# merlresearch/tssep

Measured on AMD Instinct MI355X. Metric: frames/sec fwd+bwd, 4-spk TS-SEP, 16kHz 4s chunks, higher is better.
Workload: dtype bf16x3+f32

## Files before the change

include/tssep_hip.h:

```cpp
#ifndef TSSEP_HIP_H
#define TSSEP_HIP_H

#include <stdint.h>

#ifdef __cplusplus
extern "C" {
#endif

#define TSSEP_OK 0
#define TSSEP_E_SHAPE (-1)
#define TSSEP_E_ALIGN (-2)
#define TSSEP_E_UNSUPPORTED (-3)
#define TSSEP_E_LAUNCH (-4)
#define TSSEP_E_NULL (-5)

int tssep_abi_version(void);
const char* tssep_arch(void);

int tssep_probe_mfma(float* out_4x4, float* out_32x32, void* stream);
int tssep_probe_xcc(int* out, int nblocks, void* stream);
int tssep_probe_clock(int64_t* out, int nblocks, int iters, int heavy, void* stream);
int tssep_probe_rewrite(float* buf, int nblocks, int bytes_per_wg, int reps, int flavour, int read_flavour,
                        const float* stream_src, int64_t stream_bytes, int pressure, float* sink, void* stream);

// ... 6 lines not shown
                   float* X, int64_t T, void* stream);

int64_t tssep_istft_chunks(int64_t N);
int tssep_istft_fwd(const float* X, int64_t rows, int64_t T, int size, int shift,
                    int fading, const float* wsyn, const float* tw,
                    float* y, int64_t N, const float* tgt, float* abs_partial, void* stream);
int tssep_istft_bwd(const float* dy, int64_t rows, int64_t N, int size, int shift,
                    int fading, const float* wsyn, const float* tw,
                    float* dX, int64_t T, void* stream);

int tssep_mask_istft_fwd(const float* logit, const float* obs, int64_t B, int64_t K, int64_t T,
                         int size, int shift, int fading, const float* wsyn, const float* tw,
                         float* y, int64_t N, const float* tgt, float* abs_partial, void* stream);
int tssep_mask_istft_bwd(const float* dy, const float* logit, const float* obs, int64_t B,
                         int64_t K, int64_t N, int size, int shift, int fading,
                         const float* wsyn, const float* tw, float* dlogit, int64_t T, void* stream);
int tssep_mask_istft_bwd_loss(const float* est, const float* tgt, const float* sums, const float* gout,
                              const float* logit, const float* obs, int64_t B, int64_t K, int64_t N,
                              int size, int shift, int fading, const float* wsyn, const float* tw,
                              const int32_t* iperm, int bt_major, float* dlogit, int64_t T, void* stream);
int tssep_mask_istft_gated_fwd(const float* logit, const float* obs, int64_t B, int64_t K, int64_t T, int size,
                               int shift, int fading, const float* wsyn, const float* tw, float* y, int64_t N,
                               const float* tgt, float* abs_partial, void* stream);
int tssep_mask_istft_gated_bwd(const float* est, const float* tgt, const float* sums, const float* gout,
                               const float* vad, const float* gout_vad, const float* logit, const float* obs,
                               int64_t B, int64_t K, int64_t N, int size, int shift, int fading,
                               const float* wsyn, const float* tw, const int32_t* iperm, int bt_major,
                               float* dlogit, int64_t T, void* stream);

int64_t tssep_feat_workspace_bytes(int64_t B, int64_t T, int n_mels, int F, int stat_axis);
int tssep_feat_fwd(const float* X, int64_t B, int64_t T, int F,
                   const float* fb, const float* dct, int n_mels, int n_mfcc,
                   float top_db, int stat_axis, float* out, int64_t ld_out, void* ws, void* stream);

typedef struct tssep_gemm_args {
  const float* A; const float* B; float* C;
  int64_t M, N, K;
  int64_t lda, ldb, ldc;
  int32_t a_kmajor, b_kmajor;
  int64_t b_kshift, kperiod;
  const float* bias;
  int32_t act;
  int32_t accumulate;
  int32_t c_remap;
  int64_t c_T, c_K, c_sb, c_sk, c_st, c_cm, c_co;
  const int32_t* c_perm; int64_t c_perm_ld;
  int32_t splitk; int64_t c_split_stride;
  int32_t precision;
  int32_t b_ones_col;
  const float* aux; int64_t ldaux;
} tssep_gemm_args;
int tssep_gemm_f32(const tssep_gemm_args* args, void* stream);

#define TSSEP_GEMM_AUTO 0
#define TSSEP_GEMM_F32 1
#define TSSEP_GEMM_PIPE 2
#define TSSEP_GEMM_TALL2 3
#define TSSEP_GEMM_TALL4 4
#define TSSEP_GEMM_TALL4_XCOL 5
#define TSSEP_GEMM_BIG 6
#define TSSEP_GEMM_STREAM 7
#define TSSEP_GEMM_NT_W160 8
#define TSSEP_GEMM_TN 9
#define TSSEP_GEMM_TN_TALL 10
#define TSSEP_GEMM_TN_BIG 11
#define TSSEP_GEMM_TN_W160 12
// ... 174 lines not shown
```

tssep_amd/csrc/feat.hip:

```cpp
#include <math.h>
#include "common.h"

namespace {

__device__ __forceinline__ unsigned ord(float f) {
  const unsigned u = __float_as_uint(f);
  return (u & 0x80000000u) ? ~u : (u | 0x80000000u);
}
__device__ __forceinline__ float unord(unsigned u) {
  return __uint_as_float((u & 0x80000000u) ? (u & 0x7fffffffu) : ~u);
}

constexpr int MAXF = 1032;
constexpr int GSLOTS = 64;

struct FeatWs {
  unsigned* gmax;
  unsigned* umax;
  int* range;
  float* fbT;
  float* db;
};
constexpr int STAT_TF = 0, STAT_T = 1, STAT_F = 2;
__host__ __device__ inline int64_t feat_nmax(int64_t B, int F, int stat) { return stat == STAT_T ? B * F : B; }
__host__ __device__ inline FeatWs feat_ws(void* ws, int64_t B , int n_mels) {
  FeatWs w;
  char* p = (char*)ws;
  w.gmax = (unsigned*)p;
  w.umax = (unsigned*)(p + GSLOTS * 4);
  const int64_t off1 = GSLOTS * 4 + ((B * 4 + 15) / 16) * 16;
  w.range = (int*)(p + off1);
  const int64_t off2 = off1 + (((int64_t)2 * n_mels * 4 + 15) / 16) * 16;
  w.fbT = (float*)(p + off2);
  w.db = (float*)(p + off2 + (int64_t)n_mels * MAXF * 4);
  return w;
}

__global__ __launch_bounds__(64) void feat_init_kernel(void* ws, int64_t B, const float* __restrict__ fb,
                                                       int F, int n_mels) {
  FeatWs w = feat_ws(ws, B, n_mels);
  const int lane = threadIdx.x, m = blockIdx.x;
  if (m == 0) w.gmax[lane] = 0u;
  for (int64_t b = (int64_t)m * 64 + lane; b < B; b += (int64_t)gridDim.x * 64) w.umax[b] = 0u;
  if (m >= n_mels) return;
  float lo = (float)F, hi = 0.f;
  for (int f = lane; f < F; f += 64) {
    const float v = fb[(int64_t)f * n_mels + m];
    w.fbT[(int64_t)m * MAXF + f] = v;
    if (v != 0.f) { lo = fminf(lo, (float)f); hi = fmaxf(hi, (float)(f + 1)); }
  }
  lo = -wave_max(-lo);
  hi = wave_max(hi);
  if (lane == 0) {
    w.range[2 * m] = hi == 0.f ? 0 : (int)lo;
    w.range[2 * m + 1] = (int)hi;
  }
}

constexpr int FPW = 4;
constexpr int CWMAX = 2 * MAXF;
constexpr int LMELS = 128;

__global__ __launch_bounds__(256) void feat_pass1_kernel(const float2* __restrict__ X, int64_t B,
                                                         int64_t T, int F,
                                                         const float* __restrict__ fb, int n_mels,
                                                         int n_mfcc, void* ws, int stat, int log_mels) {
  __shared__ float pw[4][MAXF];
  __shared__ float cw[CWMAX];
  __shared__ int clo[LMELS], chi[LMELS], coff[LMELS + 1];
  __shared__ int s_packed;
  FeatWs w = feat_ws(ws, feat_nmax(B, F, stat), n_mels);
  const int tid = threadIdx.x, lane = tid & 63, wave = tid >> 6;
  if (n_mfcc > 0) {
    if (tid < n_mels && tid < LMELS) {
      clo[tid] = w.range[2 * tid];
      chi[tid] = w.range[2 * tid + 1];
    }
    __syncthreads();
    if (tid == 0) {
      int tot = 0;
      const int nm = n_mels < LMELS ? n_mels : LMELS;
      for (int m = 0; m < nm; ++m) {
        coff[m] = tot;
        const int wd = chi[m] - clo[m];
        tot += wd > 0 ? wd : 0;
      }
      coff[nm] = tot;
      s_packed = (n_mels <= LMELS && tot <= CWMAX) ? 1 : 0;
    }
    __syncthreads();
    if (s_packed)
      for (int m = wave; m < n_mels; m += 4)
        for (int f = clo[m] + lane; f < chi[m]; f += 64) cw[coff[m] + f - clo[m]] = w.fbT[(int64_t)m * MAXF + f];
    __syncthreads();
  }
  const bool packed = n_mfcc > 0 && s_packed;
  float dbmax = -INFINITY;
  for (int it = 0; it < FPW; ++it) {
    const int64_t frame = ((int64_t)blockIdx.x * FPW + it) * 4 + wave;
    if (frame >= B * T) break;
    const float2* x = X + frame * F;
    float amax = 0.f;
    float2 xv[17];
#pragma unroll
    for (int r = 0; r < 17; ++r) {
      const int f = lane + 64 * r;
      xv[r] = f < F ? x[f] : make_float2(0.f, 0.f);
    }
#pragma unroll
    for (int r = 0; r < 17; ++r) {
      const int f = lane + 64 * r;
      if (f < F) {
        const float p = xv[r].x * xv[r].x + xv[r].y * xv[r].y;
        pw[wave][f] = p;
        amax = fmaxf(amax, sqrtf(p));
        if (stat == STAT_T) {
          unsigned* slot = w.umax + (frame / T) * F + f;
          const unsigned o_ = ord(sqrtf(p));
          if (o_ > __hip_atomic_load(slot, __ATOMIC_RELAXED, __HIP_MEMORY_SCOPE_AGENT)) atomicMax(slot, o_);
        }
      }
    }
    __builtin_amdgcn_fence(__ATOMIC_RELEASE, "wavefront");
    __builtin_amdgcn_wave_barrier();
    __builtin_amdgcn_fence(__ATOMIC_ACQUIRE, "wavefront");
    amax = wave_max(amax);
    if (lane == 0 && stat == STAT_TF) atomicMax(w.umax + frame / T, ord(amax));
    if (n_mfcc > 0) {
      for (int m0 = 0; m0 < n_mels; m0 += 64) {
        float mine = 0.f;
        const int mm = n_mels - m0 < 64 ? n_mels - m0 : 64;
        if (lane < mm) {
          const int m = m0 + lane;
          const int lo = packed ? clo[m] : w.range[2 * m], hi = packed ? chi[m] : w.range[2 * m + 1];
          const float* frow = packed ? cw + coff[m] - lo : w.fbT + (int64_t)m * MAXF;
          const float* prow = pw[wave];
          float s0 = 0.f, s1 = 0.f, s2 = 0.f, s3 = 0.f;
          int f = lo;
          for (; f + 3 < hi; f += 4) {
            s0 = fmaf(prow[f], frow[f], s0);
            s1 = fmaf(prow[f + 1], frow[f + 1], s1);
            s2 = fmaf(prow[f + 2], frow[f + 2], s2);
            s3 = fmaf(prow[f + 3], frow[f + 3], s3);
          }
          if (f < hi) s0 = fmaf(prow[f], frow[f], s0);
          if (f + 1 < hi) s1 = fmaf(prow[f + 1], frow[f + 1], s1);
          if (f + 2 < hi) s2 = fmaf(prow[f + 2], frow[f + 2], s2);
          mine = (s0 + s1) + (s2 + s3);
        }
        if (lane < mm) {
          const float db = log_mels ? logf(mine + 1e-6f) : 10.0f * log10f(fmaxf(mine, 1e-10f));
          w.db[frame * n_mels + m0 + lane] = db;
          dbmax = fmaxf(dbmax, db);
        }
      }
    }
    __builtin_amdgcn_fence(__ATOMIC_RELEASE, "wavefront");
    __builtin_amdgcn_wave_barrier();
    __builtin_amdgcn_fence(__ATOMIC_ACQUIRE, "wavefront");
  }
  if (n_mfcc > 0) {
    dbmax = wave_max(dbmax);
    if (lane == 0 && dbmax > -INFINITY) atomicMax(w.gmax + (blockIdx.x & (GSLOTS - 1)), ord(dbmax));
  }
}

__global__ __launch_bounds__(256) void feat_pass2_kernel(const float2* __restrict__ X, int64_t B,
                                                         int64_t T, int F,
                                                         const float* __restrict__ dct, int n_mels,
                                                         int n_mfcc, float top_db,
                                                         float* __restrict__ out, int64_t ld_out,
                                                         const void* ws, int stat) {
  __shared__ float dbl[4][64];
  FeatWs w = feat_ws(const_cast<void*>(ws), feat_nmax(B, F, stat), n_mels);
  const int lane = threadIdx.x & 63, wave = threadIdx.x >> 6;
  const int64_t frame = (int64_t)blockIdx.x * 4 + wave;
  const bool valid = frame < B * T;
  float* o = out + (valid ? frame : 0) * ld_out;
  if (n_mfcc > 0) {
    const float floor_db = top_db < 0.f ? -INFINITY : wave_max(unord(w.gmax[lane])) - top_db;
    for (int m0 = 0; m0 < n_mels; m0 += 64) {
      if (valid && m0 + lane < n_mels)
        dbl[wave][lane] = fmaxf(w.db[frame * n_mels + m0 + lane], floor_db);
      __syncthreads();
      if (valid) {
        const int mm = n_mels - m0 < 64 ? n_mels - m0 : 64;
        for (int c = lane; c < n_mfcc; c += 64) {
          float s = m0 ? o[c] : 0.f;
          for (int m = 0; m < mm; ++m) s = fmaf(dbl[wave][m], dct[(int64_t)(m0 + m) * n_mfcc + c], s);
          o[c] = s;
        }
      }
      __syncthreads();
    }
  }
  if (!valid) return;
  const float2* x = X + frame * F;
  float2 xv[17];
#pragma unroll
  for (int r = 0; r < 17; ++r) {
    const int f = lane + 64 * r;
    xv[r] = f < F ? x[f] : make_float2(0.f, 0.f);
  }
  if (stat == STAT_TF) {
    const float scale = (float)(M_E - 1.0) / unord(w.umax[frame / T]);
#pragma unroll
    for (int r = 0; r < 17; ++r) {
      const int f = lane + 64 * r;
      if (f < F) o[n_mfcc + f] = log1pf(sqrtf(xv[r].x * xv[r].x + xv[r].y * xv[r].y) * scale);
    }
    return;
  }
  float fmx = 0.f;
  if (stat == STAT_F) {
#pragma unroll
    for (int r = 0; r < 17; ++r)
      if (lane + 64 * r < F) fmx = fmaxf(fmx, sqrtf(xv[r].x * xv[r].x + xv[r].y * xv[r].y));
    fmx = wave_max(fmx);
  }
#pragma unroll
  for (int r = 0; r < 17; ++r) {
    const int f = lane + 64 * r;
    if (f < F) {
      const float norm = stat == STAT_F ? fmx : unord(w.umax[(frame / T) * F + f]);
      o[n_mfcc + f] = log1pf(sqrtf(xv[r].x * xv[r].x + xv[r].y * xv[r].y) * ((float)(M_E - 1.0) / norm));
    }
  }
}

}

extern "C" int64_t tssep_feat_workspace_bytes(int64_t B, int64_t T, int n_mels, int F, int stat_axis) {
  if (stat_axis < 0 || stat_axis > 2 || F <= 0) return 0;
  FeatWs w = feat_ws(nullptr, feat_nmax(B, F, stat_axis), n_mels);
  return (int64_t)((char*)w.db - (char*)nullptr) + B * T * (int64_t)n_mels * 4 + 16;
}

extern "C" int tssep_feat_fwd(const float* X, int64_t B, int64_t T, int F, const float* fb,
                              const float* dct, int n_mels, int n_mfcc, float top_db, int stat_axis,
                              float* out, int64_t ld_out, void* ws, void* stream) {
  if (!X || !out || !ws) return TSSEP_E_NULL;
  if (n_mfcc > 0 && (!fb || !dct)) return TSSEP_E_NULL;
  if (B <= 0 || T <= 0 || F <= 0 || F > MAXF || ld_out < n_mfcc + F) return TSSEP_E_SHAPE;
  if (n_mfcc > 0 && (n_mels <= 0 || n_mels > 1024)) return TSSEP_E_SHAPE;
  if (n_mfcc == 0) n_mels = 0;
  if (stat_axis < 0 || stat_axis > 2) return TSSEP_E_SHAPE;
  if ((((uintptr_t)X) & 7u) || (((uintptr_t)ws) & 15u)) return TSSEP_E_ALIGN;
  hipStream_t s = (hipStream_t)stream;
  const int nm = n_mels > 0 ? n_mels : 1;
  const int64_t nmax = feat_nmax(B, F, stat_axis);
  const int64_t nb0 = (nmax + 64 * 16 - 1) / (64 * 16);
  hipLaunchKernelGGL(feat_init_kernel, dim3((unsigned)(nb0 > nm ? (nb0 > 4096 ? 4096 : nb0) : nm)), dim3(64), 0, s, ws, nmax, fb, F, n_mels);
  const unsigned blocks = (unsigned)((B * T + 3) / 4);
  const unsigned blocks1 = (unsigned)((B * T + 4 * FPW - 1) / (4 * FPW));
  hipLaunchKernelGGL(feat_pass1_kernel, dim3(blocks1), dim3(256), 0, s, (const float2*)X, B, T, F,
                     fb, n_mels, n_mfcc, ws, stat_axis, top_db < 0.f ? 1 : 0);
  hipLaunchKernelGGL(feat_pass2_kernel, dim3(blocks), dim3(256), 0, s, (const float2*)X, B, T, F,
                     dct, n_mels, n_mfcc, top_db, out, ld_out, ws, stat_axis);
  return tssep_launch_status();
}
```

tssep_amd/csrc/stft.hip:

```cpp
#include <math.h>
#include "common.h"

namespace {

typedef __amdgpu_buffer_rsrc_t srd_t;
typedef unsigned u32x2_t __attribute__((ext_vector_type(2)));
__device__ __forceinline__ srd_t make_srd(const void* p, int64_t bytes) {
  return __builtin_amdgcn_make_buffer_rsrc(const_cast<void*>(p), 0, (int)(bytes > 0x7fffffff ? 0x7fffffff : bytes), 0x00020000);
}
__device__ __forceinline__ float2 bload2(srd_t r, unsigned voff) {
  const u32x2_t v = __builtin_amdgcn_raw_buffer_load_b64(r, (int)voff, 0, 0);
  return make_float2(__uint_as_float(v[0]), __uint_as_float(v[1]));
}

__device__ __forceinline__ float bload1(srd_t r, unsigned voff) {
  return __uint_as_float(__builtin_amdgcn_raw_buffer_load_b32(r, (int)voff, 0, 0));
}
__device__ __forceinline__ void bstore1(srd_t r, unsigned voff, float v) {
  __builtin_amdgcn_raw_buffer_store_b32(__float_as_uint(v), r, (int)voff, 0, 0);
}

constexpr int NH = 512;
constexpr int LINE = NH + NH / 8;
#define PADI(i) ((i) + ((i) >> 3))
#define WAVE_SYNC()                                          \
  do {                                                       \
    __builtin_amdgcn_fence(__ATOMIC_RELEASE, "wavefront");   \
    __builtin_amdgcn_wave_barrier();                         \
    __builtin_amdgcn_fence(__ATOMIC_ACQUIRE, "wavefront");   \
  } while (0)

__device__ __forceinline__ float2 cmul(float2 a, float2 b) {
  return make_float2(a.x * b.x - a.y * b.y, a.x * b.y + a.y * b.x);
}
// ... 36 lines not shown

__device__ __forceinline__ void fft512_wave(float2 (&v)[8], float2* buf, const float2* twl, int lane) {
  fft8(v);
#pragma unroll
  for (int r = 0; r < 8; ++r) buf[PADI(8 * lane + r)] = v[r];
  WAVE_SYNC();
#pragma unroll
  for (int r = 0; r < 8; ++r) v[r] = buf[PADI(lane + 64 * r)];
  WAVE_SYNC();
  {
    const int k = lane & 7;
#pragma unroll
    for (int r = 1; r < 8; ++r) v[r] = cmul(v[r], twl[k * r * 8]);
    fft8(v);
    const int d = (lane >> 3) * 64 + k;
#pragma unroll
    for (int r = 0; r < 8; ++r) buf[PADI(d + 8 * r)] = v[r];
  }
  WAVE_SYNC();
#pragma unroll
  for (int r = 0; r < 8; ++r) v[r] = buf[PADI(lane + 64 * r)];
  WAVE_SYNC();
#pragma unroll
  for (int r = 1; r < 8; ++r) v[r] = cmul(v[r], twl[lane * r]);
  fft8(v);
#pragma unroll
  for (int r = 0; r < 8; ++r) buf[PADI(lane + 64 * r)] = v[r];
  WAVE_SYNC();
}

#ifndef TSSEP_RFFT_OCC
#define TSSEP_RFFT_OCC 3
#endif
template <bool MASKED, bool GATED = false>
__global__ __launch_bounds__(256, TSSEP_RFFT_OCC) void rfft_frames_kernel(
    const float* __restrict__ x, int64_t rows, int64_t N, int64_t T, int shift, int pad_left,
    const float* __restrict__ window, const float2* __restrict__ tw, float2* __restrict__ X,
    float s_in, float s_edge, int iters, const float* __restrict__ logit,
    const float2* __restrict__ obs, float* __restrict__ dlogit, int64_t Kspk,
    const float* __restrict__ tgt, const float* __restrict__ sums, const float* __restrict__ gout,
    const int32_t* __restrict__ iperm, int bt_major, const float* __restrict__ vad = nullptr,
    const float* __restrict__ gbce = nullptr, float inv_kt = 0.f) {
  static_assert(MASKED || !GATED, "the gate belongs to the mask head");
  constexpr int LDL = NH + 1 + (GATED ? 1 : 0);
  constexpr int C0 = GATED ? 1 : 0;
  __shared__ float2 twl[NH];
  __shared__ float2 wl[NH];
  __shared__ float2 line[4][LINE];
  const int tid = threadIdx.x, lane = tid & 63;
  const int wave = __builtin_amdgcn_readfirstlane(tid >> 6);
  for (int i = tid; i < NH; i += 256) { twl[i] = tw[i]; wl[i] = reinterpret_cast<const float2*>(window)[i]; }
  __syncthreads();
  const float2 tw2_lane = tw[NH + lane];
  const int64_t total = rows * T;
  for (int it = 0; it < iters; ++it) {
    const int64_t fidx = ((int64_t)blockIdx.x * iters + it) * 4 + wave;
    const bool valid = fidx < total;
    const int64_t row = valid ? fidx / T : 0;
    const int64_t t = valid ? fidx - row * T : 0;
    const int64_t base = t * shift - pad_left;
    const float* xr = x + row * N;
    const bool lossgrad = MASKED && tgt != nullptr;
    const float* tr_ = lossgrad ? tgt + row * N : xr;
    float coef = 0.f;
    if (lossgrad) {
      const int64_t b = row / Kspk;
      coef = sums ? gout[b] / ((float)N * 2.30258509299404568402f * sums[b]) : gout[b] / (float)N;
    }
    auto lg = [&](float e, float t_) { const float d = e - t_; return d > 0.f ? coef : (d < 0.f ? -coef : 0.f); };
    const bool fast = ((N & 1) == 0) && ((base & 1) == 0) && ((((uintptr_t)x) & 7u) == 0) &&
                      (!lossgrad || (((uintptr_t)tgt) & 7u) == 0);
    float2 v[8];
    if (!valid) {
#pragma unroll
      for (int r = 0; r < 8; ++r) v[r] = make_float2(0.f, 0.f);
    } else if (fast) {
      const unsigned vo = (unsigned)((base + 2 * lane) * 4);
      const srd_t sx = make_srd(xr, N * 4);
      float2 xv[8];
#pragma unroll
      for (int r = 0; r < 8; ++r) xv[r] = bload2(sx, vo + 512u * r);
      if (lossgrad) {
        const srd_t st_ = make_srd(tr_, N * 4);
        float2 tv[8];
#pragma unroll
// ... 41 lines not shown
      for (int r = 0; r < 8; ++r) {
        ob8[r] = bload2(so, (unsigned)(lane * 8 + 512 * r));
        lg8[r] = bload1(sl, (unsigned)(C0 * 4 + lane * 4 + 256 * r));
      }
      if (GATED) lgate = bload1(sl, 0u);
    }
    fft512_wave(v, buf, twl, lane);
    if (valid) {
      float2* Xo = MASKED ? nullptr : X + fidx * (NH + 1);
      float* Dr = MASKED ? dlogit + fidx * LDL : nullptr;
      if (MASKED && bt_major) {
        const int64_t b = row / Kspk, j = row - b * Kspk;
        const int64_t kpos = iperm ? (int64_t)iperm[b * Kspk + j] : j;
        Dr = dlogit + ((b * T + t) * Kspk + kpos) * LDL;
      }
      const float gm = GATED ? sigmoidf_mask(lgate) : 1.f;
      float gpart = 0.f;
      auto emit = [&](int k, float2 o, float lgk, float2 ob) {
        if (GATED) {
          const float s = sigmoidf_mask(lgk);
          const float dm = ob.x * o.x + ob.y * o.y;
          Dr[C0 + k] = dm * gm * s * (1.0f - s);
          gpart += dm * s;
        } else if (MASKED) {
          const float m = sigmoidf_mask(lgk);
          Dr[k] = (ob.x * o.x + ob.y * o.y) * m * (1.0f - m);
        } else {
          Xo[k] = o;
        }
      };
      float2 wr[8];
      lane_twiddles(tw2_lane, wr);
      const float hs_in = 0.5f * s_in;
#pragma unroll
      for (int r = 0; r < 8; ++r) {
        const int k = lane + 64 * r;
        const float2 zk = buf[PADI(k)];
        const int km = (NH - k) & (NH - 1);
        float2 zm = buf[PADI(km)];
        zm.y = -zm.y;
        const float2 u = cmul(wr[r], csub(zk, zm));
        float2 o = make_float2(zk.x + zm.x + u.y, zk.y + zm.y - u.x);
        if (k == 0) {
          o.x *= 0.5f * s_edge; o.y = 0.f;
        } else {
          o.x *= hs_in; o.y *= hs_in;
        }
        emit(k, o, MASKED ? lg8[r] : 0.f, MASKED ? ob8[r] : make_float2(0.f, 0.f));
      }
      if (lane == 0) {
        const float2 z0 = buf[0];
        emit(NH, make_float2((z0.x - z0.y) * s_edge, 0.f), MASKED ? Lr[C0 + NH] : 0.f, MASKED ? Or[NH] : make_float2(0.f, 0.f));
      }
      if (GATED) {
        const float tot = wave_sum(gpart);
        if (lane == 0) {
          float dv = tot * gm * (1.0f - gm);
          if (vad) dv += gbv * (sigmoidf_acc(lgate) - vadv) * inv_kt;
          Dr[0] = dv;
        }
      }
    }
    WAVE_SYNC();
  }
}

constexpr int RING = 7;
constexpr int HCB_MAX = 64;

#ifndef TSSEP_ISTFT_OCC
#define TSSEP_ISTFT_OCC 3
#endif
template <bool MASKED, bool GATED = false>
__global__ __launch_bounds__(256, TSSEP_ISTFT_OCC) void istft_kernel(
    const float2* __restrict__ X, int64_t T, int shift_, int64_t N,
    const float* __restrict__ wsyn, const float2* __restrict__ tw, float* __restrict__ y,
    const float* __restrict__ tgt, float* __restrict__ abs_partial, int nchunks, int hcb,
    const float* __restrict__ logit, const float2* __restrict__ obs, int64_t Kspk) {
  __shared__ float2 twl[NH];
  __shared__ float2 line[4][LINE];
  __shared__ __attribute__((aligned(16))) float fr[RING][1024];
  __shared__ float red[4];
  static_assert(MASKED || !GATED, "the gate belongs to the mask head");
  constexpr int LDL = NH + 1 + (GATED ? 1 : 0);
  constexpr int C0 = GATED ? 1 : 0;
  const int tid = threadIdx.x, lane = tid & 63;
  const int wave = __builtin_amdgcn_readfirstlane(tid >> 6);
  const int64_t row = blockIdx.y;
  const int c = blockIdx.x;
  for (int i = tid; i < NH; i += 256) twl[i] = tw[i];
  __syncthreads();
  const float2 tw2_lane = tw[NH + lane];
  const int64_t t_lo = (int64_t)c * hcb;
  const int64_t n0 = t_lo * 256;
  const int64_t total_hops = (N + 255) / 256;
  const int hops = (int)(total_hops - t_lo < hcb ? total_hops - t_lo : hcb);
// ... 153 lines not shown
  }
  return TSSEP_OK;
}

static int check_plan(int size, int shift) {
  if (size != 1024 || shift != 256) return TSSEP_E_UNSUPPORTED;
  return TSSEP_OK;
}
static bool generic_plan(int size, int shift) { return check_plan(size, shift) != TSSEP_OK && tssep_generic_plan_supported(size, shift); }
extern "C" int tssep_stft_plan(int size, int shift) {
  return check_plan(size, shift) == TSSEP_OK ? 1 : (tssep_generic_plan_supported(size, shift) ? 2 : 0);
}

extern "C" int tssep_stft_fwd(const float* x, int64_t rows, int64_t N, int size, int shift,
                              int fading, const float* window, const float* tw, float* X,
                              int64_t T, void* stream) {
  if (!x || !window || !tw || !X) return TSSEP_E_NULL;
  if (rows <= 0 || N <= 0 || T <= 0) return TSSEP_E_SHAPE;
  if ((((uintptr_t)X) & 7u) || (((uintptr_t)tw) & 7u) || (((uintptr_t)window) & 7u)) return TSSEP_E_ALIGN;
  if (generic_plan(size, shift))
    return tssep_generic_rfft(x, rows, N, size, shift, fading ? size - shift : 0, window, tw, X, T, 1.0f, 1.0f, stream);
  if (int e = check_plan(size, shift)) return e;
  const int iters = 4;
  const int64_t total = rows * T;
  const int64_t blocks = (total + 4 * iters - 1) / (4 * iters);
  hipLaunchKernelGGL(rfft_frames_kernel<false>, dim3((unsigned)blocks), dim3(256), 0, (hipStream_t)stream,
                     x, rows, N, T, shift, fading ? size - shift : 0, window, (const float2*)tw,
                     (float2*)X, 1.0f, 1.0f, iters, (const float*)nullptr, (const float2*)nullptr,
                     (float*)nullptr, (int64_t)1, (const float*)nullptr, (const float*)nullptr,
                     (const float*)nullptr, (const int32_t*)nullptr, 0);
  return tssep_launch_status();
}

extern "C" int tssep_istft_bwd(const float* dy, int64_t rows, int64_t N, int size, int shift,
                               int fading, const float* wsyn, const float* tw, float* dX,
                               int64_t T, void* stream) {
  if (!dy || !wsyn || !tw || !dX) return TSSEP_E_NULL;
  if (rows <= 0 || N <= 0 || T <= 0) return TSSEP_E_SHAPE;
  if ((((uintptr_t)dX) & 7u) || (((uintptr_t)tw) & 7u) || (((uintptr_t)wsyn) & 7u)) return TSSEP_E_ALIGN;
  if (generic_plan(size, shift))
    return tssep_generic_rfft(dy, rows, N, size, shift, fading ? size - shift : 0, wsyn, tw, dX, T, 2.0f / (float)size,
                              1.0f / (float)size, stream);
  if (int e = check_plan(size, shift)) return e;
  const int iters = 4;
  const int64_t total = rows * T;
  const int64_t blocks = (total + 4 * iters - 1) / (4 * iters);
  hipLaunchKernelGGL(rfft_frames_kernel<false>, dim3((unsigned)blocks), dim3(256), 0, (hipStream_t)stream,
                     dy, rows, N, T, shift, fading ? size - shift : 0, wsyn, (const float2*)tw,
                     (float2*)dX, 2.0f / (float)size, 1.0f / (float)size, iters, (const float*)nullptr,
                     (const float2*)nullptr, (float*)nullptr, (int64_t)1, (const float*)nullptr, (const float*)nullptr,
                     (const float*)nullptr, (const int32_t*)nullptr, 0);
  return tssep_launch_status();
}

extern "C" int tssep_mask_istft_bwd(const float* dy, const float* logit, const float* obs, int64_t B,
                                    int64_t K, int64_t N, int size, int shift, int fading,
                                    const float* wsyn, const float* tw, float* dlogit, int64_t T,
                                    void* stream) {
  if (!dy || !logit || !obs || !wsyn || !tw || !dlogit) return TSSEP_E_NULL;
  if (B <= 0 || K <= 0 || N <= 0 || T <= 0) return TSSEP_E_SHAPE;
  if (int e = check_plan(size, shift)) return e;
  if ((((uintptr_t)obs) & 7u) || (((uintptr_t)tw) & 7u) || (((uintptr_t)wsyn) & 7u)) return TSSEP_E_ALIGN;
  const int iters = 4;
  const int64_t rows = B * K, total = rows * T;
  const int64_t blocks = (total + 4 * iters - 1) / (4 * iters);
  hipLaunchKernelGGL(rfft_frames_kernel<true>, dim3((unsigned)blocks), dim3(256), 0, (hipStream_t)stream,
// ... 117 lines not shown
```

tssep_amd/hip_ops.py:

```python
import ctypes
import itertools
import math

import numpy as np
import torch

from . import _lib
from ._lib import GemmArgs, LstmSizes, check


KERNEL_TIMING = False
KERNEL_TIMERS = {}
KERNEL_FLOPS = {}
KERNEL_BYTES = {}


class _timed:
    def __init__(self, name, flops=0, nbytes=0):
        self.name, self.flops, self.nbytes = name, flops, nbytes

    def __enter__(self):
        if KERNEL_TIMING:
            self.s = torch.cuda.Event(enable_timing=True)
            self.e = torch.cuda.Event(enable_timing=True)
# ... 222 lines not shown
    if vad is not None:
        v, gv = _f32(vad[0]).contiguous(), _f32(vad[1]).contiguous()
        assert tuple(v.shape) == (B, K, T) and gv.numel() == B, (tuple(v.shape), (B, K, T), gv.numel())
    with _timed("maskhead_gated_bwd", 0, B * T * (8 * K * F1 + 8 * (F1 - 1)) + 4 * B * K * x.shape[-1]):
        check(L.tssep_mask_istft_gated_bwd(_p(x), _p(tgt), _p(sums), _p(gout), _p(v), _p(gv), _p(logit), _p(obs_r),
                                           B, K, x.shape[-1], size, shift, int(fading), _p(wsyn),
                                           _p(fft_tables(size, logit.device)), _p(iperm), int(bt_major), _p(dlogit),
                                           T, _stream()), "mask_istft_gated_bwd")
    return dlogit


STAT_AXES = {"tf": 0, "t": 1, "f": 2}


def feat_fwd(X, fb, dct, n_mfcc, top_db=80.0, statistics_axis="tf"):
    L = _lib.lib()
    Xr = torch.view_as_real(X.contiguous())
    B, T, F = X.shape
    n_mels = fb.shape[1] if n_mfcc else 0
    if n_mfcc:
        fb, dct = _f32(fb).contiguous(), _f32(dct).contiguous()
    D = n_mfcc + F
    ld = round_up(D, 4)
    out = torch.empty(B, T, ld, device=X.device, dtype=torch.float32)
    if ld != D:
        out[..., D:].zero_()
    stat = STAT_AXES[statistics_axis]
    ws = torch.empty(int(L.tssep_feat_workspace_bytes(B, T, max(n_mels, 1), F, stat)) // 4 + 4,
                     device=X.device, dtype=torch.float32)
    check(L.tssep_feat_fwd(_p(Xr), B, T, F, _p(fb) if n_mfcc else None,
                           _p(dct) if n_mfcc else None, n_mels, n_mfcc, float(top_db), stat, _p(out),
                           ld, _p(ws), _stream()), "feat_fwd")
    return out[..., :D], ld


GEMM_PRECISION = "bf16x3"
_PREC = {"f32": 0, "bf16x3": 1, "bf16": 3}


def _gemm_args(A, lda, B, ldb, C, ldc, M, N, K, a_kmajor=False, b_kmajor=False, bias=None, act=0,
               accumulate=False, b_kshift=0, kperiod=0, remap=None, splitk=1, split_stride=0,
               b_ones_col=False, aux=None):
    def ptr(x):
        if isinstance(x, tuple):
            return x[0].data_ptr() + 4 * x[1]
        return x.data_ptr()
    g = GemmArgs()
    g.A, g.B, g.C = ptr(A), ptr(B), ptr(C)
    g.M, g.N, g.K = M, N, K
    g.lda, g.ldb, g.ldc = lda, ldb, ldc
    g.a_kmajor, g.b_kmajor = int(a_kmajor), int(b_kmajor)
    g.b_kshift, g.kperiod = b_kshift, kperiod
    g.bias = bias.data_ptr() if bias is not None else None
    g.act, g.accumulate = act, int(accumulate)
    if remap is not None:
        g.c_remap = 2 if remap.get("narrow") else 1
        g.c_T, g.c_K = remap["T"], remap.get("K", 1)
        g.c_sb, g.c_sk, g.c_st = remap["sb"], remap.get("sk", 0), remap["st"]
        g.c_cm, g.c_co = remap.get("cm", 0), remap.get("co", 0)
        perm = remap.get("perm")
        g.c_perm = perm.data_ptr() if perm is not None else None
        g.c_perm_ld = remap.get("perm_ld", 0)
    g.splitk, g.c_split_stride = splitk, split_stride
    g.precision = _PREC[GEMM_PRECISION]
    g.b_ones_col = int(b_ones_col)
    if act == 2:
# ... 944 lines not shown
```

Measured before the change: 2.124 million.

## Fuse feature statistics pass into the observation STFT kernel

Adds a STATS variant of the rfft frame kernel that computes per-bin power, max-abs statistics and mel dB values for the reference channel right after the FFT. This replaces the separate feat pass1 kernel, so the spectrum no longer has to be re-read from memory. A new entry point, tssep_stft_feat_fwd, and a Python wrapper chain the STFT, the stats and pass2 together. It also moves the sqrt to after the wave max and parallelises the coff prefix sum, at the cost of extra LDS and register pressure in the FFT kernel.

```diff
diff --git a/include/tssep_hip.h b/include/tssep_hip.h
--- a/include/tssep_hip.h
+++ b/include/tssep_hip.h
@@ -62,6 +62,11 @@
 int tssep_feat_fwd(const float* X, int64_t B, int64_t T, int F,
                    const float* fb, const float* dct, int n_mels, int n_mfcc,
                    float top_db, int stat_axis, float* out, int64_t ld_out, void* ws, void* stream);
+
+int tssep_stft_feat_fwd(const float* x, int64_t B, int nchan, int ref, int64_t N, int size, int shift,
+                        int fading, const float* window, const float* tw, float* X, int64_t T,
+                        const float* fb, const float* dct, int n_mels, int n_mfcc, float top_db,
+                        int stat_axis, float* out, int64_t ld_out, void* ws, void* stream);
 
 typedef struct tssep_gemm_args {
   const float* A; const float* B; float* C;
diff --git a/tssep_amd/csrc/feat.hip b/tssep_amd/csrc/feat.hip
--- a/tssep_amd/csrc/feat.hip
+++ b/tssep_amd/csrc/feat.hip
@@ -1,40 +1,7 @@
-#include <math.h>
-#include "common.h"
+#include "feat_common.h"
 
 namespace {
-
-__device__ __forceinline__ unsigned ord(float f) {
-  const unsigned u = __float_as_uint(f);
-  return (u & 0x80000000u) ? ~u : (u | 0x80000000u);
-}
-__device__ __forceinline__ float unord(unsigned u) {
-  return __uint_as_float((u & 0x80000000u) ? (u & 0x7fffffffu) : ~u);
-}
-
-constexpr int MAXF = 1032;
-constexpr int GSLOTS = 64;
-
-struct FeatWs {
-  unsigned* gmax;
-  unsigned* umax;
-  int* range;
-  float* fbT;
-  float* db;
-};
-constexpr int STAT_TF = 0, STAT_T = 1, STAT_F = 2;
-__host__ __device__ inline int64_t feat_nmax(int64_t B, int F, int stat) { return stat == STAT_T ? B * F : B; }
-__host__ __device__ inline FeatWs feat_ws(void* ws, int64_t B , int n_mels) {
-  FeatWs w;
-  char* p = (char*)ws;
-  w.gmax = (unsigned*)p;
-  w.umax = (unsigned*)(p + GSLOTS * 4);
-  const int64_t off1 = GSLOTS * 4 + ((B * 4 + 15) / 16) * 16;
-  w.range = (int*)(p + off1);
-  const int64_t off2 = off1 + (((int64_t)2 * n_mels * 4 + 15) / 16) * 16;
-  w.fbT = (float*)(p + off2);
-  w.db = (float*)(p + off2 + (int64_t)n_mels * MAXF * 4);
-  return w;
-}
+using namespace feat;
 
 __global__ __launch_bounds__(64) void feat_init_kernel(void* ws, int64_t B, const float* __restrict__ fb,
                                                        int F, int n_mels) {
@@ -58,43 +25,17 @@
 }
 
 constexpr int FPW = 4;
-constexpr int CWMAX = 2 * MAXF;
-constexpr int LMELS = 128;
 
 __global__ __launch_bounds__(256) void feat_pass1_kernel(const float2* __restrict__ X, int64_t B,
                                                          int64_t T, int F,
                                                          const float* __restrict__ fb, int n_mels,
                                                          int n_mfcc, void* ws, int stat, int log_mels) {
   __shared__ float pw[4][MAXF];
-  __shared__ float cw[CWMAX];
-  __shared__ int clo[LMELS], chi[LMELS], coff[LMELS + 1];
-  __shared__ int s_packed;
+  __shared__ MelLds mel;
   FeatWs w = feat_ws(ws, feat_nmax(B, F, stat), n_mels);
   const int tid = threadIdx.x, lane = tid & 63, wave = tid >> 6;
-  if (n_mfcc > 0) {
-    if (tid < n_mels && tid < LMELS) {
-      clo[tid] = w.range[2 * tid];
-      chi[tid] = w.range[2 * tid + 1];
-    }
-    __syncthreads();
-    if (tid == 0) {
-      int tot = 0;
-      const int nm = n_mels < LMELS ? n_mels : LMELS;
-      for (int m = 0; m < nm; ++m) {
-        coff[m] = tot;
-        const int wd = chi[m] - clo[m];
-        tot += wd > 0 ? wd : 0;
-      }
-      coff[nm] = tot;
-      s_packed = (n_mels <= LMELS && tot <= CWMAX) ? 1 : 0;
-    }
-    __syncthreads();
-    if (s_packed)
-      for (int m = wave; m < n_mels; m += 4)
-        for (int f = clo[m] + lane; f < chi[m]; f += 64) cw[coff[m] + f - clo[m]] = w.fbT[(int64_t)m * MAXF + f];
-    __syncthreads();
-  }
-  const bool packed = n_mfcc > 0 && s_packed;
+  if (n_mfcc > 0) mel_lds_fill(mel, w, n_mels, tid);
+  const bool packed = n_mfcc > 0 && mel.packed;
   float dbmax = -INFINITY;
   for (int it = 0; it < FPW; ++it) {
     const int64_t frame = ((int64_t)blockIdx.x * FPW + it) * 4 + wave;
@@ -111,9 +52,9 @@
     for (int r = 0; r < 17; ++r) {
       const int f = lane + 64 * r;
       if (f < F) {
-        const float p = xv[r].x * xv[r].x + xv[r].y * xv[r].y;
+        const float p = power(xv[r]);
         pw[wave][f] = p;
-        amax = fmaxf(amax, sqrtf(p));
+        amax = fmaxf(amax, p);
         if (stat == STAT_T) {
           unsigned* slot = w.umax + (frame / T) * F + f;
           const unsigned o_ = ord(sqrtf(p));
@@ -124,37 +65,9 @@
     __builtin_amdgcn_fence(__ATOMIC_RELEASE, "wavefront");
     __builtin_amdgcn_wave_barrier();
     __builtin_amdgcn_fence(__ATOMIC_ACQUIRE, "wavefront");
-    amax = wave_max(amax);
+    amax = sqrtf(wave_max(amax));
     if (lane == 0 && stat == STAT_TF) atomicMax(w.umax + frame / T, ord(amax));
-    if (n_mfcc > 0) {
-      for (int m0 = 0; m0 < n_mels; m0 += 64) {
-        float mine = 0.f;
-        const int mm = n_mels - m0 < 64 ? n_mels - m0 : 64;
-        if (lane < mm) {
-          const int m = m0 + lane;
-          const int lo = packed ? clo[m] : w.range[2 * m], hi = packed ? chi[m] : w.range[2 * m + 1];
-          const float* frow = packed ? cw + coff[m] - lo : w.fbT + (int64_t)m * MAXF;
-          const float* prow = pw[wave];
-          float s0 = 0.f, s1 = 0.f, s2 = 0.f, s3 = 0.f;
-          int f = lo;
-          for (; f + 3 < hi; f += 4) {
-            s0 = fmaf(prow[f], frow[f], s0);
-            s1 = fmaf(prow[f + 1], frow[f + 1], s1);
-            s2 = fmaf(prow[f + 2], frow[f + 2], s2);
-            s3 = fmaf(prow[f + 3], frow[f + 3], s3);
-          }
-          if (f < hi) s0 = fmaf(prow[f], frow[f], s0);
-          if (f + 1 < hi) s1 = fmaf(prow[f + 1], frow[f + 1], s1);
-          if (f + 2 < hi) s2 = fmaf(prow[f + 2], frow[f + 2], s2);
-          mine = (s0 + s1) + (s2 + s3);
-        }
-        if (lane < mm) {
-          const float db = log_mels ? logf(mine + 1e-6f) : 10.0f * log10f(fmaxf(mine, 1e-10f));
-          w.db[frame * n_mels + m0 + lane] = db;
-          dbmax = fmaxf(dbmax, db);
-        }
-      }
-    }
+    if (n_mfcc > 0) dbmax = mel_db_frame(mel, packed, w, pw[wave], n_mels, log_mels, w.db + frame * n_mels, lane, dbmax);
     __builtin_amdgcn_fence(__ATOMIC_RELEASE, "wavefront");
     __builtin_amdgcn_wave_barrier();
     __builtin_amdgcn_fence(__ATOMIC_ACQUIRE, "wavefront");
@@ -170,7 +83,7 @@
                                                          const float* __restrict__ dct, int n_mels,
                                                          int n_mfcc, float top_db,
                                                          float* __restrict__ out, int64_t ld_out,
-                                                         const void* ws, int stat) {
+                                                         const void* ws, int stat, int nchan, int ref) {
   __shared__ float dbl[4][64];
   FeatWs w = feat_ws(const_cast<void*>(ws), feat_nmax(B, F, stat), n_mels);
   const int lane = threadIdx.x & 63, wave = threadIdx.x >> 6;
@@ -195,7 +108,7 @@
     }
   }
   if (!valid) return;
-  const float2* x = X + frame * F;
+  const float2* x = X + (((frame / T) * nchan + ref) * T + frame % T) * F;
   float2 xv[17];
 #pragma unroll
   for (int r = 0; r < 17; ++r) {
@@ -256,6 +169,38 @@
   hipLaunchKernelGGL(feat_pass1_kernel, dim3(blocks1), dim3(256), 0, s, (const float2*)X, B, T, F,
                      fb, n_mels, n_mfcc, ws, stat_axis, top_db < 0.f ? 1 : 0);
   hipLaunchKernelGGL(feat_pass2_kernel, dim3(blocks), dim3(256), 0, s, (const float2*)X, B, T, F,
-                     dct, n_mels, n_mfcc, top_db, out, ld_out, ws, stat_axis);
+                     dct, n_mels, n_mfcc, top_db, out, ld_out, ws, stat_axis, 1, 0);
   return tssep_launch_status();
 }
+
+int tssep_rfft_stats_launch(const float* x, int64_t rows, int64_t N, int64_t T, int shift, int pad_left, const float* window,
+                            const float* tw, float* X, const feat::StatsArgs& st, void* stream);
+
+extern "C" int tssep_stft_feat_fwd(const float* x, int64_t B, int nchan, int ref, int64_t N, int size, int shift,
+                                   int fading, const float* window, const float* tw, float* X, int64_t T,
+                                   const float* fb, const float* dct, int n_mels, int n_mfcc, float top_db,
+                                   int stat_axis, float* out, int64_t ld_out, void* ws, void* stream) {
+  constexpr int F = 513;
+  if (!x || !window || !tw || !X || !out || !ws) return TSSEP_E_NULL;
+  if (n_mfcc > 0 && (!fb || !dct)) return TSSEP_E_NULL;
+  if (size != 1024 || shift != 256) return TSSEP_E_UNSUPPORTED;
+  if (B <= 0 || nchan <= 0 || ref < 0 || ref >= nchan || N <= 0 || T <= 0 || ld_out < n_mfcc + F) return TSSEP_E_SHAPE;
+  if (n_mfcc > 0 && (n_mels <= 0 || n_mels > 1024)) return TSSEP_E_SHAPE;
+  if (n_mfcc == 0) n_mels = 0;
+  if (stat_axis < 0 || stat_axis > 2) return TSSEP_E_SHAPE;
+  if ((B * nchan * T + 15) / 16 > 0x7fffffff) return TSSEP_E_SHAPE;
+  if ((((uintptr_t)X) & 7u) || (((uintptr_t)tw) & 7u) || (((uintptr_t)window) & 7u) || (((uintptr_t)ws) & 15u))
+    return TSSEP_E_ALIGN;
+  hipStream_t s = (hipStream_t)stream;
+  const int nm = n_mels > 0 ? n_mels : 1;
+  const int64_t nmax = feat_nmax(B, F, stat_axis);
+  const int64_t nb0 = (nmax + 64 * 16 - 1) / (64 * 16);
+  hipLaunchKernelGGL(feat_init_kernel, dim3((unsigned)(nb0 > nm ? (nb0 > 4096 ? 4096 : nb0) : nm)), dim3(64), 0, s, ws, nmax, fb, F, n_mels);
+  feat::StatsArgs st;
+  st.ws = ws; st.nchan = nchan; st.ref = ref;
+  st.n_mels = n_mels; st.n_mfcc = n_mfcc; st.stat = stat_axis; st.log_mels = top_db < 0.f ? 1 : 0;
+  if (int e = tssep_rfft_stats_launch(x, B * nchan, N, T, shift, fading ? size - shift : 0, window, tw, X, st, stream)) return e;
+  hipLaunchKernelGGL(feat_pass2_kernel, dim3((unsigned)((B * T + 3) / 4)), dim3(256), 0, s, (const float2*)X, B, T, F,
+                     dct, n_mels, n_mfcc, top_db, out, ld_out, ws, stat_axis, nchan, ref);
+  return tssep_launch_status();
+}
diff --git a/tssep_amd/csrc/feat_common.h b/tssep_amd/csrc/feat_common.h
--- /dev/null
+++ b/tssep_amd/csrc/feat_common.h
@@ -0,0 +1,121 @@
+#pragma once
+#include <math.h>
+#include "common.h"
+
+namespace feat {
+
+__device__ __forceinline__ unsigned ord(float f) {
+  const unsigned u = __float_as_uint(f);
+  return (u & 0x80000000u) ? ~u : (u | 0x80000000u);
+}
+__device__ __forceinline__ float unord(unsigned u) {
+  return __uint_as_float((u & 0x80000000u) ? (u & 0x7fffffffu) : ~u);
+}
+
+__device__ __forceinline__ float power(float2 v) {
+#pragma clang fp contract(off)
+  const float a = v.x * v.x, b = v.y * v.y;
+  return a + b;
+}
+
+constexpr int MAXF = 1032;
+constexpr int GSLOTS = 64;
+
+struct FeatWs {
+  unsigned* gmax;
+  unsigned* umax;
+  int* range;
+  float* fbT;
+  float* db;
+};
+constexpr int STAT_TF = 0, STAT_T = 1, STAT_F = 2;
+__host__ __device__ inline int64_t feat_nmax(int64_t B, int F, int stat) { return stat == STAT_T ? B * F : B; }
+__host__ __device__ inline FeatWs feat_ws(void* ws, int64_t B , int n_mels) {
+  FeatWs w;
+  char* p = (char*)ws;
+  w.gmax = (unsigned*)p;
+  w.umax = (unsigned*)(p + GSLOTS * 4);
+  const int64_t off1 = GSLOTS * 4 + ((B * 4 + 15) / 16) * 16;
+  w.range = (int*)(p + off1);
+  const int64_t off2 = off1 + (((int64_t)2 * n_mels * 4 + 15) / 16) * 16;
+  w.fbT = (float*)(p + off2);
+  w.db = (float*)(p + off2 + (int64_t)n_mels * MAXF * 4);
+  return w;
+}
+
+constexpr int CWMAX = 2 * MAXF;
+constexpr int LMELS = 128;
+struct MelLds {
+  float cw[CWMAX];
+  int clo[LMELS], chi[LMELS], coff[LMELS + 1];
+  int packed;
+};
+
+__device__ __forceinline__ void mel_lds_fill(MelLds& L, const FeatWs& w, int n_mels, int tid) {
+  const int lane = tid & 63, wave = tid >> 6;
+  if (tid < n_mels && tid < LMELS) {
+    L.clo[tid] = w.range[2 * tid];
+    L.chi[tid] = w.range[2 * tid + 1];
+  }
+  __syncthreads();
+  {
+    const int nm = n_mels < LMELS ? n_mels : LMELS;
+    if (tid <= nm) {
+      int tot = 0;
+      for (int m = 0; m < tid; ++m) {
+        const int wd = L.chi[m] - L.clo[m];
+        tot += wd > 0 ? wd : 0;
+      }
+      L.coff[tid] = tot;
+      if (tid == nm) L.packed = (n_mels <= LMELS && tot <= CWMAX) ? 1 : 0;
+    }
+  }
+  __syncthreads();
+  if (L.packed)
+    for (int m = wave; m < n_mels; m += 4)
+      for (int f = L.clo[m] + lane; f < L.chi[m]; f += 64) L.cw[L.coff[m] + f - L.clo[m]] = w.fbT[(int64_t)m * MAXF + f];
+  __syncthreads();
+}
+
+__device__ __forceinline__ float mel_db_frame(const MelLds& L, bool packed, const FeatWs& w, const float* prow,
+                                              int n_mels, int log_mels, float* db_row, int lane, float dbmax) {
+  for (int m0 = 0; m0 < n_mels; m0 += 64) {
+    float mine = 0.f;
+    const int mm = n_mels - m0 < 64 ? n_mels - m0 : 64;
+    if (lane < mm) {
+      const int m = m0 + lane;
+      const int lo = packed ? L.clo[m] : w.range[2 * m], hi = packed ? L.chi[m] : w.range[2 * m + 1];
+      const float* frow = packed ? L.cw + L.coff[m] - lo : w.fbT + (int64_t)m * MAXF;
+      float s0 = 0.f, s1 = 0.f, s2 = 0.f, s3 = 0.f;
+      int f = lo;
+      for (; f + 3 < hi; f += 4) {
+        s0 = fmaf(prow[f], frow[f], s0);
+        s1 = fmaf(prow[f + 1], frow[f + 1], s1);
+        s2 = fmaf(prow[f + 2], frow[f + 2], s2);
+        s3 = fmaf(prow[f + 3], frow[f + 3], s3);
+      }
+      if (f < hi) s0 = fmaf(prow[f], frow[f], s0);
+      if (f + 1 < hi) s1 = fmaf(prow[f + 1], frow[f + 1], s1);
+      if (f + 2 < hi) s2 = fmaf(prow[f + 2], frow[f + 2], s2);
+      mine = (s0 + s1) + (s2 + s3);
+    }
+    if (lane < mm) {
+      const float db = log_mels ? logf(mine + 1e-6f) : 10.0f * log10f(fmaxf(mine, 1e-10f));
+      db_row[m0 + lane] = db;
+      dbmax = fmaxf(dbmax, db);
+    }
+  }
+  return dbmax;
+}
+
+__device__ __forceinline__ void raise_max(unsigned* slot, unsigned o_) {
+  if (o_ > __hip_atomic_load(slot, __ATOMIC_RELAXED, __HIP_MEMORY_SCOPE_AGENT)) atomicMax(slot, o_);
+}
+
+struct StatsArgs {
+  void* ws;
+  int nchan, ref;
+  int n_mels, n_mfcc, stat, log_mels;
+};
+
+}
diff --git a/tssep_amd/csrc/stft.hip b/tssep_amd/csrc/stft.hip
--- a/tssep_amd/csrc/stft.hip
+++ b/tssep_amd/csrc/stft.hip
@@ -1,5 +1,6 @@
 #include <math.h>
 #include "common.h"
+#include "feat_common.h"
 
 namespace {
 
@@ -102,7 +103,7 @@
 #ifndef TSSEP_RFFT_OCC
 #define TSSEP_RFFT_OCC 3
 #endif
-template <bool MASKED, bool GATED = false>
+template <bool MASKED, bool GATED = false, bool STATS = false>
 __global__ __launch_bounds__(256, TSSEP_RFFT_OCC) void rfft_frames_kernel(
     const float* __restrict__ x, int64_t rows, int64_t N, int64_t T, int shift, int pad_left,
     const float* __restrict__ window, const float2* __restrict__ tw, float2* __restrict__ X,
@@ -110,8 +111,9 @@
     const float2* __restrict__ obs, float* __restrict__ dlogit, int64_t Kspk,
     const float* __restrict__ tgt, const float* __restrict__ sums, const float* __restrict__ gout,
     const int32_t* __restrict__ iperm, int bt_major, const float* __restrict__ vad = nullptr,
-    const float* __restrict__ gbce = nullptr, float inv_kt = 0.f) {
+    const float* __restrict__ gbce = nullptr, float inv_kt = 0.f, feat::StatsArgs st = feat::StatsArgs()) {
   static_assert(MASKED || !GATED, "the gate belongs to the mask head");
+  static_assert(!(MASKED && STATS), "the statistics belong to the observation's STFT");
   constexpr int LDL = NH + 1 + (GATED ? 1 : 0);
   constexpr int C0 = GATED ? 1 : 0;
   __shared__ float2 twl[NH];
@@ -121,6 +123,21 @@
   const int wave = __builtin_amdgcn_readfirstlane(tid >> 6);
   for (int i = tid; i < NH; i += 256) { twl[i] = tw[i]; wl[i] = reinterpret_cast<const float2*>(window)[i]; }
   __syncthreads();
+  extern __shared__ __attribute__((aligned(16))) unsigned char stats_lds[];
+  feat::FeatWs fw = feat::FeatWs();
+  bool mel_packed = false;
+  float dbmax = -INFINITY, umax_run = 0.f;
+  int64_t u_run = -1;
+  if constexpr (STATS) {
+    fw = feat::feat_ws(st.ws, feat::feat_nmax(rows / st.nchan, NH + 1, st.stat), st.n_mels);
+    if (st.n_mfcc > 0) {
+      feat::mel_lds_fill(*reinterpret_cast<feat::MelLds*>(stats_lds), fw, st.n_mels, tid);
+      mel_packed = reinterpret_cast<feat::MelLds*>(stats_lds)->packed != 0;
+    }
+  }
+  auto flush_umax = [&]() {
+    if (lane == 0 && u_run >= 0) feat::raise_max(fw.umax + u_run, feat::ord(umax_run));
+  };
   const float2 tw2_lane = tw[NH + lane];
   const int64_t total = rows * T;
   for (int it = 0; it < iters; ++it) {
@@ -228,6 +245,7 @@
       float2 wr[8];
       lane_twiddles(tw2_lane, wr);
       const float hs_in = 0.5f * s_in;
+      float pr[8], pnyq = 0.f;
 #pragma unroll
       for (int r = 0; r < 8; ++r) {
         const int k = lane + 64 * r;
@@ -243,10 +261,43 @@
           o.x *= hs_in; o.y *= hs_in;
         }
         emit(k, o, MASKED ? lg8[r] : 0.f, MASKED ? ob8[r] : make_float2(0.f, 0.f));
+        if constexpr (STATS) pr[r] = feat::power(o);
       }
       if (lane == 0) {
         const float2 z0 = buf[0];
-        emit(NH, make_float2((z0.x - z0.y) * s_edge, 0.f), MASKED ? Lr[C0 + NH] : 0.f, MASKED ? Or[NH] : make_float2(0.f, 0.f));
+        const float2 on = make_float2((z0.x - z0.y) * s_edge, 0.f);
+        emit(NH, on, MASKED ? Lr[C0 + NH] : 0.f, MASKED ? Or[NH] : make_float2(0.f, 0.f));
+        if constexpr (STATS) pnyq = feat::power(on);
+      }
+      if constexpr (STATS) {
+        const int64_t u = row / st.nchan;
+        if (row - u * st.nchan == st.ref) {
+          WAVE_SYNC();
+          float* prow = reinterpret_cast<float*>(buf);
+          float amax = 0.f;
+          auto bin = [&](int k, float p) {
+            prow[k] = p;
+            amax = fmaxf(amax, p);
+            if (st.stat == feat::STAT_T) feat::raise_max(fw.umax + u * (NH + 1) + k, feat::ord(sqrtf(p)));
+          };
+#pragma unroll
+          for (int r = 0; r < 8; ++r) bin(lane + 64 * r, pr[r]);
+          if (lane == 0) bin(NH, pnyq);
+          WAVE_SYNC();
+          if (st.stat == feat::STAT_TF) {
+            amax = sqrtf(wave_max(amax));
+            if (u != u_run) {
+              flush_umax();
+              u_run = u;
+              umax_run = amax;
+            } else {
+              umax_run = fmaxf(umax_run, amax);
+            }
+          }
+          if (st.n_mfcc > 0)
+            dbmax = feat::mel_db_frame(*reinterpret_cast<const feat::MelLds*>(stats_lds), mel_packed, fw, prow, st.n_mels,
+                                       st.log_mels, fw.db + (u * T + t) * st.n_mels, lane, dbmax);
+        }
       }
       if (GATED) {
         const float tot = wave_sum(gpart);
@@ -258,6 +309,13 @@
       }
     }
     WAVE_SYNC();
+  }
+  if constexpr (STATS) {
+    flush_umax();
+    if (st.n_mfcc > 0) {
+      dbmax = wave_max(dbmax);
+      if (lane == 0 && dbmax > -INFINITY) atomicMax(fw.gmax + (blockIdx.x & (feat::GSLOTS - 1)), feat::ord(dbmax));
+    }
   }
 }
 
@@ -477,6 +535,18 @@
   return tssep_launch_status();
 }
 
+int tssep_rfft_stats_launch(const float* x, int64_t rows, int64_t N, int64_t T, int shift, int pad_left, const float* window,
+                            const float* tw, float* X, const feat::StatsArgs& st, void* stream) {
+  const int iters = 4;
+  const int64_t blocks = (rows * T + 4 * iters - 1) / (4 * iters);
+  hipLaunchKernelGGL((rfft_frames_kernel<false, false, true>), dim3((unsigned)blocks), dim3(256), sizeof(feat::MelLds),
+                     (hipStream_t)stream, x, rows, N, T, shift, pad_left, window, (const float2*)tw, (float2*)X, 1.0f, 1.0f,
+                     iters, (const float*)nullptr, (const float2*)nullptr, (float*)nullptr, (int64_t)1, (const float*)nullptr,
+                     (const float*)nullptr, (const float*)nullptr, (const int32_t*)nullptr, 0, (const float*)nullptr,
+                     (const float*)nullptr, 0.f, st);
+  return tssep_launch_status();
+}
+
 extern "C" int tssep_istft_bwd(const float* dy, int64_t rows, int64_t N, int size, int shift,
                                int fading, const float* wsyn, const float* tw, float* dX,
                                int64_t T, void* stream) {
diff --git a/tssep_amd/hip_ops.py b/tssep_amd/hip_ops.py
--- a/tssep_amd/hip_ops.py
+++ b/tssep_amd/hip_ops.py
@@ -278,6 +278,33 @@
                            _p(dct) if n_mfcc else None, n_mels, n_mfcc, float(top_db), stat, _p(out),
                            ld, _p(ws), _stream()), "feat_fwd")
     return out[..., :D], ld
+
+
+def stft_feat_fwd(x, window, fb, dct, n_mfcc, top_db=80.0, statistics_axis="tf", ref=0, size=1024, shift=256,
+                  fading=True, T=None):
+    L = _lib.lib()
+    x = _f32(x).contiguous()
+    B, C, N = x.shape
+    F = size // 2 + 1
+    if T is None:
+        T = stft_frames(N, size, shift, None, True, fading)
+    n_mels = fb.shape[1] if n_mfcc else 0
+    if n_mfcc:
+        fb, dct = _f32(fb).contiguous(), _f32(dct).contiguous()
+    D = n_mfcc + F
+    ld = round_up(D, 4)
+    X = torch.empty(B, C, T, F, 2, device=x.device, dtype=torch.float32)
+    out = torch.empty(B, T, ld, device=x.device, dtype=torch.float32)
+    if ld != D:
+        out[..., D:].zero_()
+    stat = STAT_AXES[statistics_axis]
+    ws = torch.empty(int(L.tssep_feat_workspace_bytes(B, T, max(n_mels, 1), F, stat)) // 4 + 4,
+                     device=x.device, dtype=torch.float32)
+    check(L.tssep_stft_feat_fwd(_p(x), B, C, int(ref), N, size, shift, int(fading), _p(window),
+                                _p(fft_tables(size, x.device)), _p(X), T, _p(fb) if n_mfcc else None,
+                                _p(dct) if n_mfcc else None, n_mels, n_mfcc, float(top_db), stat, _p(out), ld, _p(ws),
+                                _stream()), "stft_feat_fwd")
+    return torch.view_as_complex(X), out[..., :D], ld
 
 
 GEMM_PRECISION = "bf16x3"
```

New measurement: 2.073 million. 2.4% lower.
